# rogeliolopezcamara/prob-matrix-factorization

Measured on AMD Instinct MI355X. Metric: ratings/sec (epoch) Gaussian-MF K=64, higher is better.
Workload: dtype f32; 1 GPU; gaussian_mf_cavi_bias K=64, 1Mx100k synthetic, 50M ratings; n_items=100000, ratings_total=50000000, n_factors=64, ratings_on_rank0=50000000, users_on_rank0=1000000, parallelism=single GPU, torch_imported=False

## Files before the change

### include/pmf_hip.h

```cpp
#ifndef PMF_HIP_H
#define PMF_HIP_H

#include <stdint.h>

#ifdef __cplusplus
extern "C" {
#endif

#define PMF_ABI_VERSION 3

#define PMF_OK 0
#define PMF_EINVAL (-1)
#define PMF_EHIP (-2)
#define PMF_ENOMEM (-3)
#define PMF_ERANGE (-4)
#define PMF_ECOMM (-5)

#define PMF_F32 0
#define PMF_F64 1

#define PMF_SIDE_USER 0
#define PMF_SIDE_ITEM 1

#define PMF_ARR_FACTOR 0
// ... 8 lines not shown
#define PMF_ARR_SCALE_RATE 9
#define PMF_ARR_COUNT 10

#define PMF_KERNEL_GAMMA_SWEEP 0
#define PMF_KERNEL_GAMMA_FINAL 1
#define PMF_KERNEL_GAUSS_ACCUM 2
#define PMF_KERNEL_GAUSS_SOLVE 3
#define PMF_KERNEL_GAUSS_BIAS 4
#define PMF_KERNEL_EVAL 5
#define PMF_KERNEL_PREDICT 6
#define PMF_KERNEL_TOPK 7
#define PMF_KERNEL_GAUSS_COMBINE 8
#define PMF_KERNEL_GAUSS_SGD 9
#define PMF_KERNEL_COMM_ALLREDUCE 10
#define PMF_KERNEL_COMM_WAIT 11
#define PMF_KERNEL_COUNT 12

typedef struct pmf_ctx pmf_ctx;

int pmf_abi_version(void);
const char *pmf_last_error(void);
int pmf_device_count(int *count);

int pmf_ctx_create(int device, int64_t n_users, int64_t n_items, int n_factors, int dtype,
                   pmf_ctx **out);
int pmf_ctx_destroy(pmf_ctx *ctx);
int pmf_ctx_set_stream(pmf_ctx *ctx, void *hip_stream);
int pmf_ctx_sync(pmf_ctx *ctx);

int pmf_ctx_set_row_chunks(pmf_ctx *ctx, int side, int n_chunks);
int pmf_ctx_chunk_rows(pmf_ctx *ctx, int side, int chunk, int64_t *row_begin, int64_t *row_end);
int pmf_ctx_select_chunk(pmf_ctx *ctx, int side, int chunk);
int pmf_ctx_device_bytes(pmf_ctx *ctx, int64_t *bytes);

int pmf_ctx_set_ratings(pmf_ctx *ctx, int64_t nnz, const int32_t *user_ids,
                        const int32_t *item_ids, const double *ratings);

int pmf_set_array(pmf_ctx *ctx, int side, int array, const double *host);
int pmf_get_array(pmf_ctx *ctx, int side, int array, double *host);
int pmf_get_array_rows(pmf_ctx *ctx, int side, int array, int64_t n, const int64_t *rows, double *host);
int pmf_set_array_rows(pmf_ctx *ctx, int side, int array, int64_t n, const int64_t *rows, const double *host);
int pmf_set_cov_identity(pmf_ctx *ctx, int side, double scale);

int pmf_gamma_sweep(pmf_ctx *ctx, int side, double shape_prior, double rate_prior,
                    int hierarchical, double hyper_shape, double hyper_rate_prior);

int pmf_gamma_ext_sweep(pmf_ctx *ctx, int side, double shape_prior, double rate_prior);

int pmf_ctx_kpad(pmf_ctx *ctx, int *kpad);
int pmf_gamma_accumulate(pmf_ctx *ctx, int side, void *stats_dev);
int pmf_gamma_finalize(pmf_ctx *ctx, int side, const void *stats_dev, double shape_prior,
                       double rate_prior, int hierarchical, double hyper_shape,
                       double hyper_rate_prior);

int pmf_gauss_factor_sweep(pmf_ctx *ctx, int side, double sigma2, double eta2);
int pmf_gauss_bias_sweep(pmf_ctx *ctx, int side, double sigma2, double eta_bias2);

int pmf_ctx_cov_stride(pmf_ctx *ctx, int *stride);
int pmf_gauss_factor_accumulate(pmf_ctx *ctx, int side, void *stats_dev);
int pmf_gauss_factor_finalize(pmf_ctx *ctx, int side, const void *stats_dev, double sigma2,
                              double eta2);
int pmf_gauss_bias_accumulate(pmf_ctx *ctx, int side, void *stats_dev);
int pmf_gauss_bias_finalize(pmf_ctx *ctx, int side, const void *stats_dev, double sigma2,
                            double eta_bias2);

#define PMF_UNIQUE_ID_BYTES 128
// ... 49 lines not shown
```

### prob-matrix-factorization_amd/csrc/pmf_ctx.hip

```cpp
#include <limits.h>
#include <stdarg.h>
#include <stdlib.h>
#include <stdio.h>
#include <string.h>

#include <algorithm>
#include <exception>
#include <new>

#include "pmf_internal.h"

static thread_local char g_err[512] = "";

void pmf_set_error(const char *fmt, ...) {
    va_list ap;
    va_start(ap, fmt);
    vsnprintf(g_err, sizeof(g_err), fmt, ap);
    va_end(ap);
}

extern "C" const char *pmf_last_error(void) { return g_err; }
extern "C" int pmf_abi_version(void) { return PMF_ABI_VERSION; }

extern "C" int pmf_device_count(int *count) {
// ... 113 lines not shown
    PMF_HIP_CHECK(hipGetDeviceCount(&ndev));
    PMF_REQUIRE(device >= 0 && device < ndev, PMF_EINVAL, "pmf_ctx_create: device %d of %d", device, ndev);
    PMF_HIP_CHECK(hipSetDevice(device));
    hipDeviceProp_t prop;
    PMF_HIP_CHECK(hipGetDeviceProperties(&prop, device));
    PMF_REQUIRE(strncmp(prop.gcnArchName, "gfx950", 6) == 0, PMF_EINVAL,
                "pmf_ctx_create: device %d is %s; this library is built for gfx950 only", device,
                prop.gcnArchName);
    pmf_ctx *ctx = new (std::nothrow) pmf_ctx();
    PMF_REQUIRE(ctx, PMF_ENOMEM, "pmf_ctx_create: out of host memory");
    ctx->device = device;
    ctx->dtype = dtype;
    ctx->elem = dtype == PMF_F64 ? 8 : 4;
    ctx->rows[0] = n_users;
    ctx->rows[1] = n_items;
    ctx->K = n_factors;
    ctx->kpad = (n_factors + PMF_VEC - 1) / PMF_VEC * PMF_VEC;
    {
        const int line = 128 / (int)ctx->elem;
        if ((ctx->kpad % line) * (int)ctx->elem > 64) ctx->kpad = (ctx->kpad + line - 1) / line * line;
    }
    ctx->kp = n_factors * (n_factors + 1) / 2;
    ctx->cov_stride = (ctx->kp + PMF_VEC - 1) / PMF_VEC * PMF_VEC;
    hipError_t e = hipStreamCreateWithFlags(&ctx->own_stream, hipStreamNonBlocking);
    if (e != hipSuccess) {
        pmf_set_error("hipStreamCreate failed: %s", hipGetErrorString(e));
        delete ctx;
        return PMF_EHIP;
    }
    ctx->stream = ctx->own_stream;
    ctx->gauss_generic = getenv("PMF_GAUSS_GENERIC") != nullptr;
    ctx->gauss_unfused = getenv("PMF_GAUSS_UNFUSED") != nullptr;
    ctx->gauss_lds_solve = getenv("PMF_GAUSS_LDS_SOLVE") != nullptr;
    ctx->topk_two_phase = getenv("PMF_TOPK_TWO_PHASE") != nullptr;
    if (const char *nb = getenv("PMF_TOPK_STAGE_BUFFERS")) ctx->topk_stage_buffers = atoi(nb);
    if (const char *mb = getenv("PMF_TOPK_MAX_BLOCKS")) ctx->topk_max_blocks = atoi(mb);
    if (const char *ex = getenv("PMF_COMM_EXCHANGE")) {
        if (!strcmp(ex, "allreduce")) ctx->exchange = PMF_EXCHANGE_ALLREDUCE;
        else if (!strcmp(ex, "scatter_gather")) ctx->exchange = PMF_EXCHANGE_SCATTER_GATHER;
    }
    *out = ctx;
    return PMF_OK;
}

static void free_tasks(pmf_ctx *ctx, PmfTaskList &t) {
    pmf_dev_free(ctx, t.d_tasks, (size_t)t.n_tasks * sizeof(PmfTask));
    pmf_dev_free(ctx, t.d_split, (size_t)t.n_split * sizeof(PmfSplitRow));
    pmf_dev_free(ctx, t.d_split_rows, (size_t)t.n_split * sizeof(int32_t));
    t = PmfTaskList();
}

static void free_index(pmf_ctx *ctx) {
    for (int s = 0; s < 2; ++s) {
        PmfSideIndex &ix = ctx->index[s];
        pmf_dev_free(ctx, ix.d_ptr, (size_t)(ctx->rows[s] + 1) * sizeof(int64_t));
        pmf_dev_free(ctx, ix.d_other, (size_t)ctx->nnz * sizeof(int32_t));
        pmf_dev_free(ctx, ix.d_val, (size_t)ctx->nnz * ctx->elem);
        ix.d_ptr = nullptr;
        ix.d_other = nullptr;
        ix.d_val = nullptr;
        pmf_dev_free(ctx, ix.d_nonempty, (size_t)ix.n_nonempty * sizeof(int32_t));
        ix.d_nonempty = nullptr;
        ix.n_nonempty = 0;
        ix.h_ptr.clear();
        ix.h_nonempty.clear();
        ix.nonempty_off.clear();
        free_tasks(ctx, ix.gamma_tasks);
        free_tasks(ctx, ix.gauss_tasks);
        free_tasks(ctx, ix.bias_tasks);
        free_tasks(ctx, ix.sgd_tasks);
    }
    ctx->nnz = 0;
}

static void free_eval(pmf_ctx *ctx) {
    PmfEvalSet &ev = ctx->eval;
    pmf_dev_free(ctx, ev.d_u, (size_t)ev.n * 4);
    pmf_dev_free(ctx, ev.d_i, (size_t)ev.n * 4);
    pmf_dev_free(ctx, ev.d_y, (size_t)ev.n * 8);
    pmf_dev_free(ctx, ev.d_label, (size_t)ev.n * 4);
    ev = PmfEvalSet();
}

extern "C" int pmf_ctx_destroy(pmf_ctx *ctx) {
    if (!ctx) return PMF_OK;
    (void)hipSetDevice(ctx->device);
    (void)hipStreamSynchronize(ctx->stream);
    pmf_comm_release(ctx);
    for (auto &r : ctx->prof_pending) {
        (void)hipEventDestroy(r.a);
        (void)hipEventDestroy(r.b);
    }
    for (auto &e : ctx->prof_pool) (void)hipEventDestroy(e);
    free_index(ctx);
    free_eval(ctx);
    for (int s = 0; s < 2; ++s)
        for (int a = 0; a < PMF_ARR_COUNT; ++a)
            if (ctx->arr[s][a]) pmf_dev_free(ctx, ctx->arr[s][a], pmf_array_elems(ctx, s, a) * ctx->elem);
    pmf_dev_free(ctx, ctx->d_partial, ctx->partial_bytes);
    pmf_dev_free(ctx, ctx->d_scratch, ctx->scratch_bytes);
    if (ctx->h_pinned) (void)hipHostFree(ctx->h_pinned);
    (void)hipStreamDestroy(ctx->own_stream);
    delete ctx;
    return PMF_OK;
}

extern "C" int pmf_ctx_set_stream(pmf_ctx *ctx, void *hip_stream) {
    CHECK_CTX(ctx, "pmf_ctx_set_stream");
    PMF_HIP_CHECK(hipSetDevice(ctx->device));
    PMF_HIP_CHECK(hipStreamSynchronize(ctx->stream));
    ctx->stream = hip_stream ? (hipStream_t)hip_stream : ctx->own_stream;
    return PMF_OK;
}

extern "C" int pmf_ctx_sync(pmf_ctx *ctx) {
    CHECK_CTX(ctx, "pmf_ctx_sync");
    PMF_HIP_CHECK(hipSetDevice(ctx->device));
    if (pmf_comm_active(ctx)) return pmf_comm_wait_stream(ctx, ctx->stream, "pmf_ctx_sync");
    PMF_HIP_CHECK(hipStreamSynchronize(ctx->stream));
    return PMF_OK;
}

extern "C" int pmf_ctx_device_bytes(pmf_ctx *ctx, int64_t *bytes) {
    CHECK_CTX(ctx, "pmf_ctx_device_bytes");
    PMF_REQUIRE(bytes, PMF_EINVAL, "pmf_ctx_device_bytes: null argument");
    *bytes = ctx->device_bytes;
    return PMF_OK;
}

extern "C" int pmf_ctx_kpad(pmf_ctx *ctx, int *kpad) {
    CHECK_CTX(ctx, "pmf_ctx_kpad");
    PMF_REQUIRE(kpad, PMF_EINVAL, "pmf_ctx_kpad: null argument");
    *kpad = ctx->kpad;
    return PMF_OK;
}

extern "C" int pmf_ctx_cov_stride(pmf_ctx *ctx, int *stride) {
    CHECK_CTX(ctx, "pmf_ctx_cov_stride");
    PMF_REQUIRE(stride, PMF_EINVAL, "pmf_ctx_cov_stride: null argument");
    *stride = ctx->cov_stride;
    return PMF_OK;
}

static void build_tasks(const std::vector<int64_t> &ptr, int64_t rows, int chunk, bool keep_empty,
                        const std::vector<int64_t> &row_bounds, std::vector<PmfTask> &tasks,
                        std::vector<PmfSplitRow> &split, int64_t &n_slots, std::vector<int64_t> &task_off,
                        std::vector<int64_t> &split_off) {
    std::vector<PmfTask> raw;
    raw.reserve((size_t)rows + 1024);
    n_slots = 0;
    for (int64_t r = 0; r < rows; ++r) {
        int64_t n = ptr[r + 1] - ptr[r];
        if (n == 0 && !keep_empty) continue;
        if (n <= chunk) {
            raw.push_back(PmfTask{ptr[r], (int32_t)r, (int32_t)n, -1, 0});
            continue;
        }
        int64_t q = (n + chunk - 1) / chunk;
        int64_t base = n / q, extra = n % q, at = ptr[r];
// ... 99 lines not shown
        PMF_HIP_CHECK(hipMemcpy(out.d_split, split.data(), split.size() * sizeof(PmfSplitRow), hipMemcpyHostToDevice));
        std::vector<int32_t> ids(split.size());
        for (size_t k = 0; k < split.size(); ++k) ids[k] = split[k].row;
        PMF_HIP_CHECK(hipMemcpy(out.d_split_rows, ids.data(), ids.size() * sizeof(int32_t), hipMemcpyHostToDevice));
    }
    return PMF_OK;
}

static int build_work_lists(pmf_ctx *ctx, int side) {
    PmfSideIndex &ix = ctx->index[side];
    const int64_t rows = ctx->rows[side];
    free_tasks(ctx, ix.gamma_tasks);
    free_tasks(ctx, ix.gauss_tasks);
    free_tasks(ctx, ix.bias_tasks);
    free_tasks(ctx, ix.sgd_tasks);
    const std::vector<int64_t> bounds = chunk_bounds(ctx, side);
    ix.nonempty_off.assign(bounds.size(), (int64_t)ix.h_nonempty.size());
    for (size_t g = 0; g + 1 < bounds.size(); ++g)
        ix.nonempty_off[g] = std::lower_bound(ix.h_nonempty.begin(), ix.h_nonempty.end(), (int32_t)bounds[g]) -
                             ix.h_nonempty.begin();
    auto task_chunk = [&](int max_chunk) {
        int64_t c = 32;
        while (c < max_chunk && c * 65536 < ctx->nnz) c <<= 1;
        return (int)c;
    };
    int rc;
    if ((rc = upload_tasks(ctx, side, ix.h_ptr, rows, task_chunk(PMF_GAMMA_CHUNK), true, ix.gamma_tasks))) return rc;
    if ((rc = upload_tasks(ctx, side, ix.h_ptr, rows, task_chunk(PMF_GAUSS_CHUNK), false, ix.gauss_tasks))) return rc;
    if ((rc = upload_tasks(ctx, side, ix.h_ptr, rows, task_chunk(PMF_GAMMA_CHUNK), false, ix.bias_tasks))) return rc;
    if ((rc = upload_tasks(ctx, side, ix.h_ptr, rows, PMF_SGD_CHUNK, false, ix.sgd_tasks))) return rc;
    return PMF_OK;
}

static int set_ratings_impl(pmf_ctx *ctx, int64_t nnz, const int32_t *user_ids, const int32_t *item_ids,
                            const double *ratings);

extern "C" int pmf_ctx_set_ratings(pmf_ctx *ctx, int64_t nnz, const int32_t *user_ids,
                                   const int32_t *item_ids, const double *ratings) {
    try {
        return set_ratings_impl(ctx, nnz, user_ids, item_ids, ratings);
    } catch (const std::bad_alloc &) {
        pmf_set_error("pmf_ctx_set_ratings: out of host memory");
        return PMF_ENOMEM;
    } catch (const std::exception &e) {
        pmf_set_error("pmf_ctx_set_ratings: %s", e.what());
        return PMF_EINVAL;
    }
}

static int fill_side_host(pmf_ctx *ctx, int side, int64_t nnz, const int32_t *key, const int32_t *oth,
                          const double *ratings, std::vector<int32_t> &other, std::vector<char> &val) {
    const int64_t rows = ctx->rows[side];
    PmfSideIndex &ix = ctx->index[side];
    ix.h_ptr.assign((size_t)rows + 1, 0);
    for (int64_t n = 0; n < nnz; ++n) ix.h_ptr[(size_t)key[n] + 1]++;
    for (int64_t r = 0; r < rows; ++r) ix.h_ptr[(size_t)r + 1] += ix.h_ptr[(size_t)r];
    std::vector<int64_t> cursor(ix.h_ptr.begin(), ix.h_ptr.end() - 1);
    pmf_with_dtype(ctx, [&](auto t) {
        auto *v = (decltype(t) *)val.data();
        for (int64_t n = 0; n < nnz; ++n) {
            int64_t d = cursor[(size_t)key[n]]++;
            other[(size_t)d] = oth[n];
            v[d] = (decltype(t))ratings[n];
        }
    });
    PMF_HIP_CHECK(hipMemcpy(ix.d_ptr, ix.h_ptr.data(), (size_t)(rows + 1) * sizeof(int64_t), hipMemcpyHostToDevice));
// ... 37 lines not shown
    free_index(ctx);
    ctx->nnz = nnz;
    for (int side = 0; side < 2; ++side) {
        PmfSideIndex &ix = ctx->index[side];
        rc = pmf_dev_alloc(ctx, (void **)&ix.d_ptr, (size_t)(ctx->rows[side] + 1) * sizeof(int64_t));
        if (!rc) rc = pmf_dev_alloc(ctx, (void **)&ix.d_other, (size_t)nnz * sizeof(int32_t));
        if (!rc) rc = pmf_dev_alloc(ctx, &ix.d_val, (size_t)nnz * ctx->elem);
        if (rc) {
            pmf_index_device_abort(build);
            return rc;
        }
    }
    if (on_host) {
        std::vector<int32_t> other((size_t)nnz);
        std::vector<char> val((size_t)nnz * ctx->elem);
        if ((rc = fill_side_host(ctx, PMF_SIDE_USER, nnz, user_ids, item_ids, ratings, other, val))) return rc;
        if ((rc = fill_side_host(ctx, PMF_SIDE_ITEM, nnz, item_ids, user_ids, ratings, other, val))) return rc;
    } else {
        if ((rc = pmf_index_device_finish(ctx, build, nnz))) return rc;
    }
    for (int side = 0; side < 2; ++side) {
        const int64_t rows = ctx->rows[side];
        PmfSideIndex &ix = ctx->index[side];
        std::vector<int32_t> nonempty;
        for (int64_t r = 0; r < rows; ++r)
            if (ix.h_ptr[(size_t)r + 1] > ix.h_ptr[(size_t)r]) nonempty.push_back((int32_t)r);
        ix.n_nonempty = (int64_t)nonempty.size();
        if ((rc = pmf_dev_alloc(ctx, (void **)&ix.d_nonempty, nonempty.size() * sizeof(int32_t)))) return rc;
        if (!nonempty.empty())
            PMF_HIP_CHECK(hipMemcpy(ix.d_nonempty, nonempty.data(), nonempty.size() * sizeof(int32_t), hipMemcpyHostToDevice));
        ix.h_nonempty.swap(nonempty);
        if ((rc = build_work_lists(ctx, side))) return rc;
    }
    return PMF_OK;
}

static int set_row_chunks_impl(pmf_ctx *ctx, int side, int n_chunks) {
    CHECK_CTX(ctx, "pmf_ctx_set_row_chunks");
    PMF_REQUIRE(side == PMF_SIDE_USER || side == PMF_SIDE_ITEM, PMF_EINVAL, "pmf_ctx_set_row_chunks: bad side %d", side);
    PMF_REQUIRE(n_chunks >= 1 && n_chunks <= 1024, PMF_EINVAL,
                "pmf_ctx_set_row_chunks: n_chunks = %d outside [1, 1024]", n_chunks);
    if ((int64_t)n_chunks > ctx->rows[side]) n_chunks = (int)(ctx->rows[side] > 0 ? ctx->rows[side] : 1);
    PMF_HIP_CHECK(hipSetDevice(ctx->device));
    PMF_HIP_CHECK(hipStreamSynchronize(ctx->stream));
    ctx->n_chunks[side] = n_chunks;
    ctx->cur_chunk[side] = -1;
    if (ctx->index[side].d_ptr) return build_work_lists(ctx, side);
    return PMF_OK;
}

extern "C" int pmf_ctx_set_row_chunks(pmf_ctx *ctx, int side, int n_chunks) {
    try {
        return set_row_chunks_impl(ctx, side, n_chunks);
    } catch (const std::bad_alloc &) {
        pmf_set_error("pmf_ctx_set_row_chunks: out of host memory");
        return PMF_ENOMEM;
    }
}

extern "C" int pmf_ctx_chunk_rows(pmf_ctx *ctx, int side, int chunk, int64_t *row_begin, int64_t *row_end) {
    CHECK_CTX(ctx, "pmf_ctx_chunk_rows");
    PMF_REQUIRE(side == PMF_SIDE_USER || side == PMF_SIDE_ITEM, PMF_EINVAL, "pmf_ctx_chunk_rows: bad side %d", side);
    PMF_REQUIRE(row_begin && row_end, PMF_EINVAL, "pmf_ctx_chunk_rows: null argument");
    PMF_REQUIRE(chunk >= 0 && chunk < ctx->n_chunks[side], PMF_ERANGE,
                "pmf_ctx_chunk_rows: chunk %d outside [0, %d)", chunk, ctx->n_chunks[side]);
    *row_begin = pmf_chunk_row0(ctx, side, chunk);
    *row_end = pmf_chunk_row0(ctx, side, chunk + 1);
// ... 327 lines not shown
```

### prob-matrix-factorization_amd/csrc/pmf_gauss.hip

```cpp
#include <stdlib.h>

#include <algorithm>
#include <type_traits>

#include "pmf_device.h"

typedef float f32x16 __attribute__((ext_vector_type(16)));

template <typename T>
struct GaussParams {
    const PmfTask *tasks;
    int64_t n_tasks;
    const PmfSplitRow *split;
    const int32_t *other;
    const T *val;
    const T *factor_other;
    const T *cov_other;
    const T *bias_self;
    const T *bias_other;
    T *partial;
    T *dst_s;
    int64_t dst_s_stride;
    T *dst_w;
    int64_t dst_w_stride;
    int K, kpad, kp, cov_stride;
};

__device__ __forceinline__ void wave_lds_fence() {
    __builtin_amdgcn_fence(__ATOMIC_ACQ_REL, "wavefront");
    __builtin_amdgcn_wave_barrier();
}

__device__ __forceinline__ int rfl(int x) { return __builtin_amdgcn_readfirstlane(x); }

__device__ __forceinline__ PmfTask load_task_uniform(const PmfTask *tasks, int64_t id) {
    PmfTask t = tasks[id];
    PmfTask r;
    r.row = rfl(t.row);
    r.len = rfl(t.len);
    r.slot = rfl(t.slot);
    r.pad = 0;
    unsigned lo = (unsigned)rfl((int)(t.start & 0xFFFFFFFFll)), hi = (unsigned)rfl((int)(t.start >> 32));
    r.start = (int64_t)(((unsigned long long)hi << 32) | lo);
    return r;
}

__device__ __forceinline__ void tri_rc(int p, int &r, int &c) {
    r = (int)((sqrtf(8.0f * (float)p + 1.0f) - 1.0f) * 0.5f);
    while ((r + 1) * (r + 2) / 2 <= p) ++r;
    while (r * (r + 1) / 2 > p) --r;
    c = p - r * (r + 1) / 2;
}

template <typename T, int KR>
__device__ __forceinline__ void solve_from_image(const T *img, T wj, int K, int kpad, T inv_sigma2, T inv_eta2,
                                                 T *vout, T *mout, int lane);

template <typename T, int KS = 0>
// ... 578 lines not shown
                reinterpret_cast<float4 *>(img)[q] = mm;
            }
        }
        __syncthreads();
        pair_solve_mfma<MT>(img, xbuf, gbuf, wbuf, K, kpad, stride, inv_sigma2, inv_eta2,
                            cov_self + (int64_t)t.row * stride, factor_self + (int64_t)t.row * kpad, wave, lane);
        return;
    }
    float *out_s, *out_w;
    if (t.slot >= 0) {
        out_s = p.partial + (int64_t)t.slot * (stride + kpad);
        out_w = out_s + stride;
    } else {
        out_s = p.dst_s + (int64_t)t.row * p.dst_s_stride;
        out_w = p.dst_w + (int64_t)t.row * p.dst_w_stride;
    }
#pragma unroll
    for (int s = 0; s < NT; ++s) {
        const int q = q_begin + lane + 64 * s;
        if (q < q_end) {
            const float4 mm = reinterpret_cast<const float4 *>(img)[q];
            float4 o = acc[s];
            o.x += mm.x;
            o.y += mm.y;
            o.z += mm.z;
            o.w += mm.w;
            reinterpret_cast<float4 *>(out_s)[q] = o;
        }
    }
    const int jj = threadIdx.x;
    if (jj < kpad) out_w[jj] = jj < K ? wbuf[jj] : 0.f;
}

template <int KB, int NT, bool FUSE, int KS = KB>
__global__ __launch_bounds__(256, KB == 64 ? 2 : 3) void gauss_accum_mfma_kernel(GaussParams<float> p, float inv_sigma2,
                                                                                float inv_eta2, float *cov_self,
                                                                                float *factor_self) {
    constexpr int NB = KB == 64 ? 3 : 1;
    constexpr int PU = NT >= 5 ? 1 : (NT >= 3 ? 2 : (NT == 2 ? 4 : 8));
    extern __shared__ __align__(16) unsigned char smem_raw[];
    const int wave = threadIdx.x >> 6, lane = threadIdx.x & 63;
    const int64_t task_id = (int64_t)blockIdx.x * 4 + wave;
    if (task_id >= p.n_tasks) return;
    const PmfTask t = load_task_uniform(p.tasks, task_id);
    const int h = lane >> 5, c = lane & 31;
    const int K = p.K, kpad = p.kpad, stride = p.cov_stride, chunks = p.cov_stride / PMF_VEC;
    const int32_t *col = p.other + t.start;
    const float *val = p.val + t.start;
    const float b_self = p.bias_self ? p.bias_self[t.row] : 0.f;
    const bool lo_ok = c < K, hi_ok = (KB == 64) && (32 + c < K);

    f32x16 d[NB];
#pragma unroll
    for (int b = 0; b < NB; ++b)
#pragma unroll
        for (int r = 0; r < 16; ++r) d[b][r] = 0.f;
    float4 acc[NT];
#pragma unroll
    for (int s = 0; s < NT; ++s) acc[s] = make_float4(0.f, 0.f, 0.f, 0.f);
    float wlo = 0.f, whi = 0.f;

    int idx_b = 0;
    float val_b = 0.f;
    auto trip = [&](int j, auto full_tag) {
        constexpr bool FULL = decltype(full_tag)::value;
        float4 a[PU][NT], b[PU][NT];
        float mlo[PU], mhi[PU], res[PU];
        if ((j & 63) == 0) {
            const int jj = min(j + lane, t.len - 1);
            idx_b = col[jj];
            val_b = val[jj];
        }
#pragma unroll
        for (int u = 0; u < PU; ++u) {
            const int j0 = j + 2 * u, l0 = j0 & 63;
            const bool has0 = FULL || j0 < t.len, has1 = FULL || j0 + 1 < t.len;
            const int o0 = __builtin_amdgcn_readlane(idx_b, l0);
            const int o1 = __builtin_amdgcn_readlane(idx_b, l0 + 1);
            const float x0 = __builtin_bit_cast(float, __builtin_amdgcn_readlane(__builtin_bit_cast(int, val_b), l0));
            const float x1 = __builtin_bit_cast(float, __builtin_amdgcn_readlane(__builtin_bit_cast(int, val_b), l0 + 1));
            const int oh = h ? o1 : o0;
            const bool live = h ? has1 : has0;
            const float *mrow = p.factor_other + (int64_t)oh * kpad;
            mlo[u] = (live && lo_ok) ? mrow[c] : 0.f;
            mhi[u] = (live && hi_ok) ? mrow[32 + c] : 0.f;
            const float xh = h ? x1 : x0;
            res[u] = live ? xh - b_self - (p.bias_other ? p.bias_other[oh] : 0.f) : 0.f;
            const float4 *v0 = reinterpret_cast<const float4 *>(p.cov_other + (int64_t)o0 * stride);
            const float4 *v1 = reinterpret_cast<const float4 *>(p.cov_other + (int64_t)o1 * stride);
#pragma unroll
            for (int s = 0; s < NT; ++s) {
                const int q = (s + 1 < NT) ? lane + 64 * s : min(lane + 64 * s, chunks - 1);
                a[u][s] = make_float4(0.f, 0.f, 0.f, 0.f);
                b[u][s] = make_float4(0.f, 0.f, 0.f, 0.f);
                if (has0) a[u][s] = v0[q];
                if (has1) b[u][s] = v1[q];
            }
        }
#pragma unroll
        for (int u = 0; u < PU; ++u) {
            wlo = fmaf(mlo[u], res[u], wlo);
            whi = fmaf(mhi[u], res[u], whi);
            d[0] = __builtin_amdgcn_mfma_f32_32x32x2f32(mlo[u], mlo[u], d[0], 0, 0, 0);
            if constexpr (KB == 64) {
                d[1] = __builtin_amdgcn_mfma_f32_32x32x2f32(mhi[u], mlo[u], d[1], 0, 0, 0);
                d[2] = __builtin_amdgcn_mfma_f32_32x32x2f32(mhi[u], mhi[u], d[2], 0, 0, 0);
            }
#pragma unroll
            for (int s = 0; s < NT; ++s) {
                acc[s].x += a[u][s].x + b[u][s].x;
                acc[s].y += a[u][s].y + b[u][s].y;
                acc[s].z += a[u][s].z + b[u][s].z;
                acc[s].w += a[u][s].w + b[u][s].w;
            }
        }
    };
    int j = 0;
    for (; j + 2 * PU <= t.len; j += 2 * PU) trip(j, std::true_type{});
    if (j < t.len) trip(j, std::false_type{});

    float *img = reinterpret_cast<float *>(smem_raw) + (int64_t)wave * stride;
    for (int q = lane; q < chunks; q += 64) reinterpret_cast<float4 *>(img)[q] = make_float4(0.f, 0.f, 0.f, 0.f);
    wave_lds_fence();
#pragma unroll
    for (int r = 0; r < 16; ++r) {
        const int row = (r & 3) + 8 * (r >> 2) + 4 * h;
        if (row < K && c <= row) img[row * (row + 1) / 2 + c] = d[0][r];
        if constexpr (KB == 64) {
            const int R1 = 32 + row;
            if (R1 < K) {
                if (c < K) img[R1 * (R1 + 1) / 2 + c] = d[1][r];
                if (c <= row) img[R1 * (R1 + 1) / 2 + 32 + c] = d[2][r];
            }
        }
    }
    wave_lds_fence();
    wlo += __shfl_xor(wlo, 32, 64);
    whi += __shfl_xor(whi, 32, 64);
    if (FUSE && t.slot < 0) {
#pragma unroll
        for (int s = 0; s < NT; ++s) {
            const int q = lane + 64 * s;
            if (q < chunks) {
                float4 m = reinterpret_cast<float4 *>(img)[q];
                m.x += acc[s].x;
                m.y += acc[s].y;
                m.z += acc[s].z;
                m.w += acc[s].w;
                reinterpret_cast<float4 *>(img)[q] = m;
            }
        }
        wave_lds_fence();
// ... 326 lines not shown
            return true;
        }
    }
    hipLaunchKernelGGL((gauss_accum_generic_kernel<T, 0>), grid, dim3(256), plain, ctx->stream, p, (T)0, (T)0,
                       (T *)nullptr, (T *)nullptr);
    return false;
}

template <typename T>
static int run_factor_accumulate(pmf_ctx *ctx, int side, PmfPass pass, void *stats, double sigma2, double eta2,
                                 bool *fused = nullptr) {
    const int other = 1 - side;
    const PmfSideIndex &ix = ctx->index[side];
    const bool acc = pass == PMF_PASS_ACCUMULATE;
    const PmfTaskView tl = pmf_task_view(ctx, side, ix.gauss_tasks, acc);
    int rc;
    PMF_REQUIRE(ix.d_ptr, PMF_EINVAL, "pmf_gauss_factor_sweep: ratings have not been set");
    if ((rc = pmf_require_array(ctx, side, PMF_ARR_FACTOR, "pmf_gauss_factor_sweep"))) return rc;
    if ((rc = pmf_require_array(ctx, side, PMF_ARR_COV, "pmf_gauss_factor_sweep"))) return rc;
    if ((rc = pmf_require_array(ctx, other, PMF_ARR_FACTOR, "pmf_gauss_factor_sweep"))) return rc;
    if ((rc = pmf_require_array(ctx, other, PMF_ARR_COV, "pmf_gauss_factor_sweep"))) return rc;
    const int width = ctx->cov_stride + ctx->kpad;
    if (tl.n_slots > 0 && (rc = pmf_ensure_partial(ctx, (size_t)tl.n_slots * width * sizeof(T)))) return rc;
    if (acc && tl.row1 > tl.row0)
        PMF_HIP_CHECK(hipMemsetAsync((T *)stats + tl.row0 * width, 0, (size_t)(tl.row1 - tl.row0) * width * sizeof(T), ctx->stream));
    GaussParams<T> p;
    p.tasks = tl.d_tasks;
    p.n_tasks = tl.n_tasks;
    p.split = tl.d_split;
    p.other = ix.d_other;
    p.val = (const T *)ix.d_val;
    p.factor_other = (const T *)ctx->arr[other][PMF_ARR_FACTOR];
    p.cov_other = (const T *)ctx->arr[other][PMF_ARR_COV];
    const bool bias = pmf_has_bias(ctx);
    p.bias_self = bias ? (const T *)ctx->arr[side][PMF_ARR_BIAS] : nullptr;
    p.bias_other = bias ? (const T *)ctx->arr[other][PMF_ARR_BIAS] : nullptr;
    p.partial = (T *)ctx->d_partial;
    p.dst_s = acc ? (T *)stats : (T *)ctx->arr[side][PMF_ARR_COV];
    p.dst_s_stride = acc ? width : ctx->cov_stride;
    p.dst_w = acc ? (T *)stats + ctx->cov_stride : (T *)ctx->arr[side][PMF_ARR_FACTOR];
    p.dst_w_stride = acc ? width : ctx->kpad;
    p.K = ctx->K;
    p.kpad = ctx->kpad;
    p.kp = ctx->kp;
    p.cov_stride = ctx->cov_stride;
    bool solved = false;
    if (tl.n_tasks > 0) {
        PmfProfScope prof(ctx, PMF_KERNEL_GAUSS_ACCUM);
        const bool fuse = !acc && !ctx->gauss_unfused;
        const T is2 = (T)(1.0 / sigma2), ie2 = (T)(1.0 / eta2);
        if (std::is_same<T, float>::value && !ctx->gauss_generic && ctx->K <= 128) {
            if constexpr (std::is_same<T, float>::value) solved = launch_accum_mfma_fp32(ctx, p, tl.n_tasks, fuse, is2, ie2);
        } else {
            solved = launch_accum_generic(ctx, p, tl.n_tasks, fuse && ctx->K <= 64, is2, ie2);
        }
    }
    if (fused) *fused = solved;
    if (tl.n_split > 0) {
        PmfProfScope prof(ctx, PMF_KERNEL_GAUSS_COMBINE);
        hipLaunchKernelGGL((gauss_combine_kernel<T>), dim3((unsigned)tl.n_split), dim3(256), 0, ctx->stream, p);
    }
    PMF_HIP_CHECK(hipGetLastError());
    return PMF_OK;
}

template <typename T>
// ... 181 lines not shown
```

### prob-matrix-factorization_amd/csrc/pmf_internal.h

```cpp
#pragma once

#include <hip/hip_runtime.h>
#include <stdint.h>

#include <functional>
#include <string>
#include <type_traits>
#include <vector>

#include "pmf_hip.h"

#ifndef PMF_TRANSPORT_HOSTSHM
#define PMF_TRANSPORT_HOSTSHM 1
#endif

#define PMF_WAVE 64
#define PMF_VEC 4
#define PMF_RATE_FLOOR 1e-10
#define PMF_MAX_LABELS 32

void pmf_set_error(const char *fmt, ...);

#define PMF_HIP_CHECK(expr)                                                         \
    do {                                                                            \
// ... 39 lines not shown
    int64_t n_tasks = 0;
    int64_t n_slots = 0;
    int64_t n_split = 0;
    int32_t max_len = 0;
    PmfTask *d_tasks = nullptr;
    PmfSplitRow *d_split = nullptr;
    int32_t *d_split_rows = nullptr;
    std::vector<int64_t> task_off, split_off;
};

struct PmfTaskView {
    const PmfTask *d_tasks = nullptr;
    const PmfSplitRow *d_split = nullptr;
    const int32_t *d_split_rows = nullptr;
    int64_t n_tasks = 0, n_split = 0, n_slots = 0;
    int64_t row0 = 0, row1 = 0;
    const int32_t *d_nonempty = nullptr;
    int64_t n_nonempty = 0;
};

struct PmfSideIndex {
    int64_t *d_ptr = nullptr;
    int32_t *d_other = nullptr;
    void *d_val = nullptr;
    std::vector<int64_t> h_ptr;
    int32_t *d_nonempty = nullptr;
    int64_t n_nonempty = 0;
    std::vector<int32_t> h_nonempty;
    std::vector<int64_t> nonempty_off;
    PmfTaskList gamma_tasks;
    PmfTaskList gauss_tasks;
    PmfTaskList bias_tasks;
    PmfTaskList sgd_tasks;
};

struct PmfEvalSet {
    int64_t n = 0;
    int n_labels = 0;
    int32_t *d_u = nullptr;
    int32_t *d_i = nullptr;
    double *d_y = nullptr;
    int32_t *d_label = nullptr;
};

struct pmf_ctx {
    int device = 0;
    int dtype = PMF_F32;
    int64_t rows[2] = {0, 0};
    int K = 0;
    int kpad = 0;
    int kp = 0;
    int cov_stride = 0;
    int64_t nnz = 0;
    hipStream_t own_stream = nullptr;
    hipStream_t stream = nullptr;
    size_t elem = 4;

    int n_chunks[2] = {1, 1};
    int cur_chunk[2] = {-1, -1};
    int64_t fin_row0 = -1, fin_row1 = -1;
    int exchange = PMF_EXCHANGE_AUTO;

    void *arr[2][PMF_ARR_COUNT] = {};
    PmfSideIndex index[2];
    PmfEvalSet eval;

    void *d_partial = nullptr;
    size_t partial_bytes = 0;
    void *d_scratch = nullptr;
    size_t scratch_bytes = 0;
    void *h_pinned = nullptr;
    size_t pinned_bytes = 0;

    int64_t device_bytes = 0;

    bool gauss_generic = false;
    bool gauss_unfused = false;
    bool gauss_lds_solve = false;
    int topk_max_blocks = 0;
    int topk_stage_buffers = 0;
    bool topk_two_phase = false;

    struct PmfComm *comm = nullptr;
    void *d_stats[2] = {nullptr, nullptr};
    size_t stats_bytes[2] = {0, 0};

    bool prof = false;
    struct ProfRec {
        hipEvent_t a, b;
        int kernel;
    };
    std::vector<ProfRec> prof_pending;
    std::vector<hipEvent_t> prof_pool;
    double prof_ms[PMF_KERNEL_COUNT] = {};
    int64_t prof_n[PMF_KERNEL_COUNT] = {};
};

#define PMF_GAMMA_CHUNK 512
#define PMF_SGD_CHUNK 256
#define PMF_GAUSS_CHUNK 512

static inline int64_t pmf_chunk_row0(const pmf_ctx *ctx, int side, int c) {
    return ctx->rows[side] * (int64_t)c / ctx->n_chunks[side];
}
PmfTaskView pmf_task_view(const pmf_ctx *ctx, int side, const PmfTaskList &tl, bool select);

int pmf_dev_alloc(pmf_ctx *ctx, void **p, size_t bytes);
void pmf_dev_free(pmf_ctx *ctx, void *p, size_t bytes);
int pmf_ensure_partial(pmf_ctx *ctx, size_t bytes);
int pmf_ensure_scratch(pmf_ctx *ctx, size_t bytes);
int pmf_ensure_pinned(pmf_ctx *ctx, size_t bytes);
size_t pmf_array_elems(const pmf_ctx *ctx, int side, int array);
int pmf_require_array(pmf_ctx *ctx, int side, int array, const char *what);
int pmf_alloc_array(pmf_ctx *ctx, int side, int array);

struct PmfIndexBuild;
int pmf_index_device_begin(pmf_ctx *ctx, int64_t nnz, const int32_t *user_ids, const int32_t *item_ids,
                           const double *ratings, PmfIndexBuild **out, int64_t *bad_position);
void pmf_index_device_abort(PmfIndexBuild *b);
int pmf_index_device_finish(pmf_ctx *ctx, PmfIndexBuild *b, int64_t nnz);

void pmf_array_shape(const pmf_ctx *ctx, int array, int *host_width, int *dev_stride);
void pmf_unpack_rows(const pmf_ctx *ctx, int array, const void *src, double *dst, int64_t rows);

bool pmf_comm_active(const pmf_ctx *ctx);
void pmf_comm_release(pmf_ctx *ctx);
int pmf_comm_wait_stream(pmf_ctx *ctx, hipStream_t stream, const char *what);
struct PmfExchange {
    bool prefer_scatter = false;
    int n_arrays = 0;
    int arrays[6] = {0, 0, 0, 0, 0, 0};
};
int pmf_comm_half_sweep(pmf_ctx *ctx, int side, int which, size_t width, bool chunked, const PmfExchange &ex,
// ... 34 lines not shown
```

### prob-matrix-factorization_amd/pmf_hip/__init__.py

```python
from __future__ import annotations

import ctypes as C
import os
import sys

import numpy as np

_HERE = os.path.dirname(os.path.abspath(__file__))
LIB_PATH = os.path.join(_HERE, "libpmf_hip.so")
TEST_LIB_PATH = os.path.join(_HERE, "libpmf_hip_test.so")
TEST_ONLY_SIGNATURES = ("pmf_comm_init_hostshm",)

F32, F64 = 0, 1
USER, ITEM = 0, 1
(ARR_FACTOR, ARR_SHAPE, ARR_RATE, ARR_PRIOR_RATE, ARR_HYPER_RATE, ARR_COV, ARR_BIAS, ARR_SCALE, ARR_SCALE_SHAPE,
 ARR_SCALE_RATE) = range(10)
PREDICT_BIAS, PREDICT_SCALE = 1, 2
KERNEL_NAMES = ("gamma_sweep", "gamma_final", "gauss_accum", "gauss_solve", "gauss_bias",
                "eval", "predict", "topk", "gauss_combine", "gauss_sgd", "comm_allreduce", "comm_wait")
UNIQUE_ID_BYTES = 128
TRANSPORT_RCCL, TRANSPORT_HOSTSHM = 0, 1
OP_SUM, OP_MAX = 0, 1
EXCHANGE = {"auto": 0, "allreduce": 1, "scatter_gather": 2}
MAX_LABELS = 32


class PmfLibraryError(RuntimeError):
    """libpmf_hip.so is missing or does not export the declared ABI."""


class PmfError(RuntimeError):
    """A C-ABI call returned a negative status."""


_p = C.c_void_p
_i32p = C.POINTER(C.c_int32)
_i64p = C.POINTER(C.c_int64)
_f64p = C.POINTER(C.c_double)

SIGNATURES = {
    "pmf_abi_version": (C.c_int, []),
    "pmf_last_error": (C.c_char_p, []),
    "pmf_device_count": (C.c_int, [C.POINTER(C.c_int)]),
    "pmf_ctx_create": (C.c_int, [C.c_int, C.c_int64, C.c_int64, C.c_int, C.c_int, C.POINTER(_p)]),
    "pmf_ctx_destroy": (C.c_int, [_p]),
    "pmf_ctx_set_stream": (C.c_int, [_p, _p]),
    "pmf_ctx_sync": (C.c_int, [_p]),
    "pmf_gauss_sgd_sweep": (C.c_int, [_p, C.c_int, C.c_double, C.c_double, C.c_double, C.c_double]),
    "pmf_ctx_sgd_stats_width": (C.c_int, [_p, C.POINTER(C.c_int)]),
    "pmf_gauss_sgd_accumulate": (C.c_int, [_p, C.c_int, _p, C.c_double, C.c_double, C.c_double, C.c_double]),
    "pmf_gauss_sgd_finalize": (C.c_int, [_p, C.c_int, _p]),
    "pmf_ctx_set_row_chunks": (C.c_int, [_p, C.c_int, C.c_int]),
    "pmf_ctx_chunk_rows": (C.c_int, [_p, C.c_int, C.c_int, C.POINTER(C.c_int64), C.POINTER(C.c_int64)]),
    "pmf_ctx_select_chunk": (C.c_int, [_p, C.c_int, C.c_int]),
    "pmf_ctx_device_bytes": (C.c_int, [_p, _i64p]),
    "pmf_ctx_set_ratings": (C.c_int, [_p, C.c_int64, _i32p, _i32p, _f64p]),
    "pmf_set_array": (C.c_int, [_p, C.c_int, C.c_int, _f64p]),
    "pmf_get_array": (C.c_int, [_p, C.c_int, C.c_int, _f64p]),
    "pmf_get_array_rows": (C.c_int, [_p, C.c_int, C.c_int, C.c_int64, _i64p, _f64p]),
    "pmf_set_array_rows": (C.c_int, [_p, C.c_int, C.c_int, C.c_int64, _i64p, _f64p]),
    "pmf_set_cov_identity": (C.c_int, [_p, C.c_int, C.c_double]),
    "pmf_gamma_sweep": (C.c_int, [_p, C.c_int, C.c_double, C.c_double, C.c_int, C.c_double, C.c_double]),
    "pmf_gamma_ext_sweep": (C.c_int, [_p, C.c_int, C.c_double, C.c_double]),
    "pmf_ctx_kpad": (C.c_int, [_p, C.POINTER(C.c_int)]),
    "pmf_gamma_accumulate": (C.c_int, [_p, C.c_int, _p]),
    "pmf_gamma_finalize": (C.c_int, [_p, C.c_int, _p, C.c_double, C.c_double, C.c_int, C.c_double, C.c_double]),
    "pmf_gauss_factor_sweep": (C.c_int, [_p, C.c_int, C.c_double, C.c_double]),
    "pmf_gauss_bias_sweep": (C.c_int, [_p, C.c_int, C.c_double, C.c_double]),
    "pmf_ctx_cov_stride": (C.c_int, [_p, C.POINTER(C.c_int)]),
    "pmf_gauss_factor_accumulate": (C.c_int, [_p, C.c_int, _p]),
    "pmf_gauss_factor_finalize": (C.c_int, [_p, C.c_int, _p, C.c_double, C.c_double]),
    "pmf_gauss_bias_accumulate": (C.c_int, [_p, C.c_int, _p]),
    "pmf_gauss_bias_finalize": (C.c_int, [_p, C.c_int, _p, C.c_double, C.c_double]),
    "pmf_predict": (C.c_int, [_p, C.c_int64, _i32p, _i32p, C.c_int, C.c_double, _f64p]),
    "pmf_eval_set": (C.c_int, [_p, C.c_int64, _i32p, _i32p, _f64p, _i32p, C.c_int]),
    "pmf_eval_run": (C.c_int, [_p, C.c_int, C.c_double, _f64p, _f64p, _i64p]),
    "pmf_topk_items": (C.c_int, [_p, C.c_int64, _i32p, C.c_int, C.c_int, _i32p, _f64p]),
    "pmf_prof_enable": (C.c_int, [_p, C.c_int]),
    "pmf_prof_reset": (C.c_int, [_p]),
    "pmf_prof_get": (C.c_int, [_p, C.c_int, _f64p, _i64p]),
    "pmf_prof_gather_ceiling": (C.c_int, [_p, C.c_int, C.c_int, _f64p]),
    "pmf_comm_unique_id": (C.c_int, [_p]),
    "pmf_comm_init": (C.c_int, [_p, C.c_int, C.c_int, _p]),
    "pmf_comm_set_exchange": (C.c_int, [_p, C.c_int]),
    "pmf_comm_attach": (C.c_int, [_p, _p]),
    "pmf_comm_destroy": (C.c_int, [_p]),
    "pmf_comm_info": (C.c_int, [_p, C.POINTER(C.c_int), C.POINTER(C.c_int), C.POINTER(C.c_int)]),
    "pmf_comm_barrier": (C.c_int, [_p]),
# ... 88 lines not shown
```

### prob-matrix-factorization_amd/pmf_hip/engine.py

```python
from __future__ import annotations

import ctypes as C

import numpy as np

from . import (ARR_COV, EXCHANGE, F32, F64, ITEM, KERNEL_NAMES, MAX_LABELS, OP_MAX, OP_SUM, TEST_LIB_PATH, UNIQUE_ID_BYTES,
               USER, PmfError, PmfLibraryError, as_f64, as_i32, check, load, ptr)


class Context:
    def __init__(self, n_users, n_items, n_factors, dtype="f32", device=0):
        self._lib = load()
        self._h = C.c_void_p()
        self.n_users, self.n_items, self.K = int(n_users), int(n_items), int(n_factors)
        self.dtype = {"f32": F32, "f64": F64, F32: F32, F64: F64}[dtype]
        self.np_dtype = np.float64 if self.dtype == F64 else np.float32
        check(self._lib.pmf_ctx_create(int(device), self.n_users, self.n_items, self.K, self.dtype,
                                       C.byref(self._h)), "pmf_ctx_create")
        k = C.c_int(0)
        check(self._lib.pmf_ctx_kpad(self._h, C.byref(k)), "pmf_ctx_kpad")
        self.kpad = k.value
        check(self._lib.pmf_ctx_cov_stride(self._h, C.byref(k)), "pmf_ctx_cov_stride")
        self.cov_stride = k.value
        self.nnz = 0
# ... 64 lines not shown
        return out

    def close(self):
        if getattr(self, "_h", None) is not None and self._h:
            self._lib.pmf_ctx_destroy(self._h)
            self._h = C.c_void_p()

    def __del__(self):
        try:
            self.close()
        except Exception:
            pass

    def __enter__(self):
        return self

    def __exit__(self, *exc):
        self.close()

    def rows(self, side):
        return self.n_users if side == USER else self.n_items

    def sync(self):
        check(self._lib.pmf_ctx_sync(self._h), "pmf_ctx_sync")

    def set_stream(self, hip_stream):
        check(self._lib.pmf_ctx_set_stream(self._h, C.c_void_p(hip_stream or 0)), "pmf_ctx_set_stream")

    def device_bytes(self):
        n = C.c_int64(0)
        check(self._lib.pmf_ctx_device_bytes(self._h, C.byref(n)), "pmf_ctx_device_bytes")
        return n.value

    def set_ratings(self, user_ids, item_ids, ratings):
        u, i, x = as_i32(user_ids, "user_ids"), as_i32(item_ids, "item_ids"), as_f64(ratings)
        if not (len(u) == len(i) == len(x)):
            raise ValueError("user_ids, item_ids and ratings must have the same length")
        check(self._lib.pmf_ctx_set_ratings(self._h, len(u), ptr(u, C.c_int32), ptr(i, C.c_int32),
                                            ptr(x, C.c_double)), "pmf_ctx_set_ratings")
        self.nnz = len(u)

    def _host_shape(self, side, array):
        r = self.rows(side)
        if array in (0, 1, 2):
            return (r, self.K)
        if array == ARR_COV:
            return (r, self.K, self.K)
        return (r,)

    def set_array(self, side, array, host):
        a = as_f64(host)
        if a.shape != self._host_shape(side, array):
            raise ValueError(f"array {array} of side {side}: expected shape "
                             f"{self._host_shape(side, array)}, got {a.shape}")
        check(self._lib.pmf_set_array(self._h, side, array, ptr(a, C.c_double)), "pmf_set_array")

    def get_array(self, side, array):
        out = np.empty(self._host_shape(side, array), dtype=np.float64)
        check(self._lib.pmf_get_array(self._h, side, array, ptr(out, C.c_double)), "pmf_get_array")
        return out

    def get_array_rows(self, side, array, rows):
        r = np.ascontiguousarray(np.asarray(rows, dtype=np.int64).reshape(-1))
        out = np.empty((len(r),) + self._host_shape(side, array)[1:], dtype=np.float64)
        check(self._lib.pmf_get_array_rows(self._h, side, array, len(r), ptr(r, C.c_int64), ptr(out, C.c_double)),
              "pmf_get_array_rows")
# ... 157 lines not shown
```

Measured before the change: 387.4 million ratings/s.

## Use nontemporal loads for cold rows to keep hot-row covariances cached

Picks the highest-degree rows on each side, up to a byte budget (default 224 MB), as 'hot' and builds a per-rating flag array marking whether the other-side row is hot. The Gaussian accumulate MFMA kernel reads these flags with a wave ballot and uses normal loads for hot rows and nontemporal loads for cold rows. The aim is to stop cold covariance and factor gathers from evicting frequently reused rows from the last-level cache. It adds an nnz-sized byte array, per-trip branching over load-policy variants, and more code size and register pressure.

```diff
diff --git a/include/pmf_hip.h b/include/pmf_hip.h
--- a/include/pmf_hip.h
+++ b/include/pmf_hip.h
@@ -64,6 +64,7 @@
 int pmf_ctx_chunk_rows(pmf_ctx *ctx, int side, int chunk, int64_t *row_begin, int64_t *row_end);
 int pmf_ctx_select_chunk(pmf_ctx *ctx, int side, int chunk);
 int pmf_ctx_device_bytes(pmf_ctx *ctx, int64_t *bytes);
+int pmf_ctx_hot_rows(pmf_ctx *ctx, int side, int32_t *rows, int64_t capacity, int64_t *n_hot);
 
 int pmf_ctx_set_ratings(pmf_ctx *ctx, int64_t nnz, const int32_t *user_ids,
                         const int32_t *item_ids, const double *ratings);
diff --git a/prob-matrix-factorization_amd/csrc/pmf_ctx.hip b/prob-matrix-factorization_amd/csrc/pmf_ctx.hip
--- a/prob-matrix-factorization_amd/csrc/pmf_ctx.hip
+++ b/prob-matrix-factorization_amd/csrc/pmf_ctx.hip
@@ -169,6 +169,8 @@
     ctx->gauss_generic = getenv("PMF_GAUSS_GENERIC") != nullptr;
     ctx->gauss_unfused = getenv("PMF_GAUSS_UNFUSED") != nullptr;
     ctx->gauss_lds_solve = getenv("PMF_GAUSS_LDS_SOLVE") != nullptr;
+    const char *hot_mb = getenv("PMF_GAUSS_HOT_MB");
+    ctx->gauss_hot_bytes = (hot_mb ? std::max(atoll(hot_mb), 0LL) : (long long)PMF_GAUSS_HOT_MB_DEFAULT) << 20;
     ctx->topk_two_phase = getenv("PMF_TOPK_TWO_PHASE") != nullptr;
     if (const char *nb = getenv("PMF_TOPK_STAGE_BUFFERS")) ctx->topk_stage_buffers = atoi(nb);
     if (const char *mb = getenv("PMF_TOPK_MAX_BLOCKS")) ctx->topk_max_blocks = atoi(mb);
@@ -200,6 +202,9 @@
         ix.d_nonempty = nullptr;
         ix.n_nonempty = 0;
         ix.h_ptr.clear();
+        pmf_dev_free(ctx, ix.d_other_hot, (size_t)ctx->nnz);
+        ix.d_other_hot = nullptr;
+        ix.h_hot.clear();
         ix.h_nonempty.clear();
         ix.nonempty_off.clear();
         free_tasks(ctx, ix.gamma_tasks);
@@ -262,6 +267,16 @@
     CHECK_CTX(ctx, "pmf_ctx_device_bytes");
     PMF_REQUIRE(bytes, PMF_EINVAL, "pmf_ctx_device_bytes: null argument");
     *bytes = ctx->device_bytes;
+    return PMF_OK;
+}
+
+extern "C" int pmf_ctx_hot_rows(pmf_ctx *ctx, int side, int32_t *rows, int64_t capacity, int64_t *n_hot) {
+    CHECK_CTX(ctx, "pmf_ctx_hot_rows");
+    PMF_REQUIRE(side == PMF_SIDE_USER || side == PMF_SIDE_ITEM, PMF_EINVAL, "pmf_ctx_hot_rows: bad side %d", side);
+    PMF_REQUIRE(n_hot && capacity >= 0 && (rows || capacity == 0), PMF_EINVAL, "pmf_ctx_hot_rows: bad argument");
+    const std::vector<int32_t> &hot = ctx->index[side].h_hot;
+    *n_hot = (int64_t)hot.size();
+    std::copy_n(hot.begin(), (size_t)std::min(capacity, *n_hot), rows);
     return PMF_OK;
 }
 
@@ -427,6 +442,48 @@
     return PMF_OK;
 }
 
+__global__ void hot_flags_kernel(const int32_t *other, const uint8_t *hot_rows, uint8_t *flags, int64_t n) {
+    for (int64_t i = blockIdx.x * (int64_t)blockDim.x + threadIdx.x; i < n; i += (int64_t)gridDim.x * blockDim.x)
+        flags[i] = hot_rows[other[i]];
+}
+
+static int build_hot_rows(pmf_ctx *ctx) {
+    if (ctx->gauss_hot_bytes <= 0 || ctx->dtype != PMF_F32 || ctx->K > 64 || ctx->nnz == 0) return PMF_OK;
+    const int64_t row_bytes = (int64_t)(ctx->cov_stride + ctx->kpad) * (int64_t)sizeof(float);
+    for (int side = 0; side < 2; ++side) {
+        PmfSideIndex &ix = ctx->index[side];
+        const int64_t n = std::min(ctx->gauss_hot_bytes / row_bytes, ix.n_nonempty);
+        std::vector<int32_t> ids(ix.h_nonempty);
+        auto deg = [&](int32_t r) { return ix.h_ptr[(size_t)r + 1] - ix.h_ptr[(size_t)r]; };
+        std::partial_sort(ids.begin(), ids.begin() + n, ids.end(), [&](int32_t a, int32_t b) {
+            return deg(a) != deg(b) ? deg(a) > deg(b) : a < b;
+        });
+        ids.resize((size_t)n);
+        ix.h_hot.swap(ids);
+    }
+    int rc;
+    for (int side = 0; side < 2; ++side) {
+        PmfSideIndex &ix = ctx->index[side];
+        const int other = 1 - side;
+        std::vector<uint8_t> mask((size_t)ctx->rows[other], 0);
+        for (int32_t r : ctx->index[other].h_hot) mask[(size_t)r] = 1;
+        uint8_t *d_mask = nullptr;
+        if ((rc = pmf_dev_alloc(ctx, (void **)&ix.d_other_hot, (size_t)ctx->nnz))) return rc;
+        if ((rc = pmf_dev_alloc(ctx, (void **)&d_mask, mask.size()))) return rc;
+        hipError_t e = hipMemcpy(d_mask, mask.data(), mask.size(), hipMemcpyHostToDevice);
+        if (e == hipSuccess) {
+            const int64_t blocks = std::min<int64_t>((ctx->nnz + 255) / 256, 65536);
+            hipLaunchKernelGGL(hot_flags_kernel, dim3((unsigned)blocks), dim3(256), 0, ctx->stream, ix.d_other, d_mask,
+                               ix.d_other_hot, ctx->nnz);
+            e = hipGetLastError();
+        }
+        if (e == hipSuccess) e = hipStreamSynchronize(ctx->stream);
+        pmf_dev_free(ctx, d_mask, mask.size());
+        PMF_HIP_CHECK(e);
+    }
+    return PMF_OK;
+}
+
 static int set_ratings_impl(pmf_ctx *ctx, int64_t nnz, const int32_t *user_ids, const int32_t *item_ids,
                             const double *ratings);
 
@@ -530,7 +587,7 @@
         ix.h_nonempty.swap(nonempty);
         if ((rc = build_work_lists(ctx, side))) return rc;
     }
-    return PMF_OK;
+    return build_hot_rows(ctx);
 }
 
 static int set_row_chunks_impl(pmf_ctx *ctx, int side, int n_chunks) {
diff --git a/prob-matrix-factorization_amd/csrc/pmf_gauss.hip b/prob-matrix-factorization_amd/csrc/pmf_gauss.hip
--- a/prob-matrix-factorization_amd/csrc/pmf_gauss.hip
+++ b/prob-matrix-factorization_amd/csrc/pmf_gauss.hip
@@ -24,6 +24,7 @@
     T *dst_w;
     int64_t dst_w_stride;
     int K, kpad, kp, cov_stride;
+    const uint8_t *hot = nullptr;
 };
 
 __device__ __forceinline__ void wave_lds_fence() {
@@ -668,6 +669,24 @@
     if (jj < kpad) out_w[jj] = jj < K ? wbuf[jj] : 0.f;
 }
 
+typedef float f32x4 __attribute__((ext_vector_type(4)));
+
+template <bool HOT>
+__device__ __forceinline__ float4 gather_ld(const float4 *ptr) {
+    if constexpr (HOT) {
+        return *ptr;
+    } else {
+        const f32x4 v = __builtin_nontemporal_load(reinterpret_cast<const f32x4 *>(ptr));
+        return make_float4(v.x, v.y, v.z, v.w);
+    }
+}
+
+template <bool HOT>
+__device__ __forceinline__ float gather_ld(const float *ptr) {
+    if constexpr (HOT) return *ptr;
+    else return __builtin_nontemporal_load(ptr);
+}
+
 template <int KB, int NT, bool FUSE, int KS = KB>
 __global__ __launch_bounds__(256, KB == 64 ? 2 : 3) void gauss_accum_mfma_kernel(GaussParams<float> p, float inv_sigma2,
                                                                                 float inv_eta2, float *cov_self,
@@ -698,15 +717,21 @@
 
     int idx_b = 0;
     float val_b = 0.f;
-    auto trip = [&](int j, auto full_tag) {
-        constexpr bool FULL = decltype(full_tag)::value;
-        float4 a[PU][NT], b[PU][NT];
-        float mlo[PU], mhi[PU], res[PU];
+    uint64_t hot_b = ~0ull;
+    const uint8_t *hot = p.hot ? p.hot + t.start : nullptr;
+    auto fetch = [&](int j) {
         if ((j & 63) == 0) {
             const int jj = min(j + lane, t.len - 1);
             idx_b = col[jj];
             val_b = val[jj];
-        }
+            if (hot) hot_b = __builtin_amdgcn_ballot_w64(__builtin_nontemporal_load(hot + jj) != 0);
+        }
+    };
+    auto trip = [&](int j, auto full_tag, auto pol_tag) {
+        constexpr bool FULL = decltype(full_tag)::value;
+        constexpr int POL = decltype(pol_tag)::value;
+        float4 a[PU][NT], b[PU][NT];
+        float mlo[PU], mhi[PU], res[PU];
 #pragma unroll
         for (int u = 0; u < PU; ++u) {
             const int j0 = j + 2 * u, l0 = j0 & 63;
@@ -718,20 +743,30 @@
             const int oh = h ? o1 : o0;
             const bool live = h ? has1 : has0;
             const float *mrow = p.factor_other + (int64_t)oh * kpad;
-            mlo[u] = (live && lo_ok) ? mrow[c] : 0.f;
-            mhi[u] = (live && hi_ok) ? mrow[32 + c] : 0.f;
             const float xh = h ? x1 : x0;
             res[u] = live ? xh - b_self - (p.bias_other ? p.bias_other[oh] : 0.f) : 0.f;
             const float4 *v0 = reinterpret_cast<const float4 *>(p.cov_other + (int64_t)o0 * stride);
             const float4 *v1 = reinterpret_cast<const float4 *>(p.cov_other + (int64_t)o1 * stride);
-#pragma unroll
-            for (int s = 0; s < NT; ++s) {
-                const int q = (s + 1 < NT) ? lane + 64 * s : min(lane + 64 * s, chunks - 1);
-                a[u][s] = make_float4(0.f, 0.f, 0.f, 0.f);
-                b[u][s] = make_float4(0.f, 0.f, 0.f, 0.f);
-                if (has0) a[u][s] = v0[q];
-                if (has1) b[u][s] = v1[q];
-            }
+            auto loads = [&](auto h0_tag, auto h1_tag) {
+                constexpr bool H0 = decltype(h0_tag)::value, H1 = decltype(h1_tag)::value;
+                mlo[u] = (live && lo_ok) ? gather_ld<H0 || H1>(mrow + c) : 0.f;
+                mhi[u] = (live && hi_ok) ? gather_ld<H0 || H1>(mrow + 32 + c) : 0.f;
+#pragma unroll
+                for (int s = 0; s < NT; ++s) {
+                    const int q = (s + 1 < NT) ? lane + 64 * s : min(lane + 64 * s, chunks - 1);
+                    a[u][s] = make_float4(0.f, 0.f, 0.f, 0.f);
+                    b[u][s] = make_float4(0.f, 0.f, 0.f, 0.f);
+                    if (has0) a[u][s] = gather_ld<H0>(v0 + q);
+                    if (has1) b[u][s] = gather_ld<H1>(v1 + q);
+                }
+            };
+            using T_ = std::true_type;
+            using F_ = std::false_type;
+            const int pol = POL >= 0 ? POL : (int)((hot_b >> l0) & 3);
+            if (pol == 3) loads(T_{}, T_{});
+            else if (pol == 2) loads(F_{}, T_{});
+            else if (pol == 1) loads(T_{}, F_{});
+            else loads(F_{}, F_{});
         }
 #pragma unroll
         for (int u = 0; u < PU; ++u) {
@@ -751,9 +786,21 @@
             }
         }
     };
+    auto run = [&](int j, auto full_tag) {
+        fetch(j);
+        if constexpr (PU > 1) {
+            trip(j, full_tag, std::integral_constant<int, -1>{});
+        } else {
+            const int pol = (int)((hot_b >> (j & 63)) & 3);
+            if (pol == 3) trip(j, full_tag, std::integral_constant<int, 3>{});
+            else if (pol == 2) trip(j, full_tag, std::integral_constant<int, 2>{});
+            else if (pol == 1) trip(j, full_tag, std::integral_constant<int, 1>{});
+            else trip(j, full_tag, std::integral_constant<int, 0>{});
+        }
+    };
     int j = 0;
-    for (; j + 2 * PU <= t.len; j += 2 * PU) trip(j, std::true_type{});
-    if (j < t.len) trip(j, std::false_type{});
+    for (; j + 2 * PU <= t.len; j += 2 * PU) run(j, std::true_type{});
+    if (j < t.len) run(j, std::false_type{});
 
     float *img = reinterpret_cast<float *>(smem_raw) + (int64_t)wave * stride;
     for (int q = lane; q < chunks; q += 64) reinterpret_cast<float4 *>(img)[q] = make_float4(0.f, 0.f, 0.f, 0.f);
@@ -1146,6 +1193,7 @@
     p.val = (const T *)ix.d_val;
     p.factor_other = (const T *)ctx->arr[other][PMF_ARR_FACTOR];
     p.cov_other = (const T *)ctx->arr[other][PMF_ARR_COV];
+    p.hot = ix.d_other_hot;
     const bool bias = pmf_has_bias(ctx);
     p.bias_self = bias ? (const T *)ctx->arr[side][PMF_ARR_BIAS] : nullptr;
     p.bias_other = bias ? (const T *)ctx->arr[other][PMF_ARR_BIAS] : nullptr;
diff --git a/prob-matrix-factorization_amd/csrc/pmf_internal.h b/prob-matrix-factorization_amd/csrc/pmf_internal.h
--- a/prob-matrix-factorization_amd/csrc/pmf_internal.h
+++ b/prob-matrix-factorization_amd/csrc/pmf_internal.h
@@ -95,6 +95,8 @@
     PmfTaskList gauss_tasks;
     PmfTaskList bias_tasks;
     PmfTaskList sgd_tasks;
+    std::vector<int32_t> h_hot;
+    uint8_t *d_other_hot = nullptr;
 };
 
 struct PmfEvalSet {
@@ -140,6 +142,7 @@
     bool gauss_generic = false;
     bool gauss_unfused = false;
     bool gauss_lds_solve = false;
+    int64_t gauss_hot_bytes = 0;
     int topk_max_blocks = 0;
     int topk_stage_buffers = 0;
     bool topk_two_phase = false;
@@ -162,6 +165,7 @@
 #define PMF_GAMMA_CHUNK 512
 #define PMF_SGD_CHUNK 256
 #define PMF_GAUSS_CHUNK 512
+#define PMF_GAUSS_HOT_MB_DEFAULT 224
 
 static inline int64_t pmf_chunk_row0(const pmf_ctx *ctx, int side, int c) {
     return ctx->rows[side] * (int64_t)c / ctx->n_chunks[side];
diff --git a/prob-matrix-factorization_amd/pmf_hip/__init__.py b/prob-matrix-factorization_amd/pmf_hip/__init__.py
--- a/prob-matrix-factorization_amd/pmf_hip/__init__.py
+++ b/prob-matrix-factorization_amd/pmf_hip/__init__.py
@@ -54,6 +54,7 @@
     "pmf_ctx_chunk_rows": (C.c_int, [_p, C.c_int, C.c_int, C.POINTER(C.c_int64), C.POINTER(C.c_int64)]),
     "pmf_ctx_select_chunk": (C.c_int, [_p, C.c_int, C.c_int]),
     "pmf_ctx_device_bytes": (C.c_int, [_p, _i64p]),
+    "pmf_ctx_hot_rows": (C.c_int, [_p, C.c_int, _i32p, C.c_int64, _i64p]),
     "pmf_ctx_set_ratings": (C.c_int, [_p, C.c_int64, _i32p, _i32p, _f64p]),
     "pmf_set_array": (C.c_int, [_p, C.c_int, C.c_int, _f64p]),
     "pmf_get_array": (C.c_int, [_p, C.c_int, C.c_int, _f64p]),
diff --git a/prob-matrix-factorization_amd/pmf_hip/engine.py b/prob-matrix-factorization_amd/pmf_hip/engine.py
--- a/prob-matrix-factorization_amd/pmf_hip/engine.py
+++ b/prob-matrix-factorization_amd/pmf_hip/engine.py
@@ -120,6 +120,14 @@
         check(self._lib.pmf_ctx_device_bytes(self._h, C.byref(n)), "pmf_ctx_device_bytes")
         return n.value
 
+    def hot_rows(self, side):
+        n = C.c_int64(0)
+        check(self._lib.pmf_ctx_hot_rows(self._h, side, None, 0, C.byref(n)), "pmf_ctx_hot_rows")
+        out = np.empty(n.value, dtype=np.int32)
+        check(self._lib.pmf_ctx_hot_rows(self._h, side, out.ctypes.data_as(C.POINTER(C.c_int32)), n.value, C.byref(n)),
+              "pmf_ctx_hot_rows")
+        return out
+
     def set_ratings(self, user_ids, item_ids, ratings):
         u, i, x = as_i32(user_ids, "user_ids"), as_i32(item_ids, "item_ids"), as_f64(ratings)
         if not (len(u) == len(i) == len(x)):
```

After: 409.2 million ratings/s (median of 6 runs). +5.6%, better.
